# dohlee/diffab-pytorch

Hardware: AMD Instinct MI355X
Metric: CDR-residue denoise-steps/sec (K=128 patch) (higher is better)
Workload: dtype f32 (bf16x6 / fp16x3 split-precision products on the 16-bit matrix cores, fp32 accumulate; fp32-accurate, DESIGN section 4)

## Files before the change

diffab-pytorch_amd/csrc/ipa_persistent.hip:

```cpp
#include "common.h"
#include "denoiser_internal.h"
#define AT_STAMP_REALTIME 1
#include "ipa_attn_tile.h"
#include "proj_frames_h3_tile.h"
#include "rowgemm_h3_tile.h"
#include "mlp_chain_tile.h"

namespace diffab {

namespace {
constexpr size_t cmax(size_t a, size_t b) { return a > b ? a : b; }
constexpr size_t kModuleLdsBytes = cmax(cmax(ipa_attn_lds_bytes(8), static_cast<size_t>(kChainLdsBytes)),
                                        cmax(static_cast<size_t>(pjh3::PJ_LDS_BYTES), static_cast<size_t>(h3tile::lds_bytes<128>())));
constexpr size_t kXImageOffset = cmax(static_cast<size_t>(pjh3::PJ_LDS_BYTES), static_cast<size_t>(h3tile::lds_bytes<128>())) / 4;
static_assert(kXImageOffset * 4 + h3tile::y_lds_bytes<128>() <= kModuleLdsBytes, "module LDS: no room for the x image of the dense phases");
static_assert(kModuleLdsBytes <= 160 * 1024, "module LDS: one work-group per CU within gfx950's 160 KiB");
static_assert(kXImageOffset % 4 == 0, "x image: 16-byte aligned rows");

struct ModuleArgs {
  float* xa;
  float* xb;
  float* proj;
  float* feat;
  const float* pair;
  const float* esc;
  const int* ctx_of_row;
  const int* last_layer_rows;
  const float* R;
  const float* t;
  const char* planes;
  size_t layer_stride, pj_off, out_off, wis_off, small_off;
  unsigned long long* stamps;
  const float* emb_X;
  MlpChainSet emb, heads;
  int B, NL;
  int stagger_ticks, stagger_classes;
};
}

__device__ __forceinline__ int module_plan_word(const int* __restrict__ plan, const int idx) {
  int w;
  asm volatile("s_load_dword %0, %1, 0x0\n\ts_waitcnt lgkmcnt(0)" : "=s"(w) : "s"(plan + idx) : "memory");
  return w;
}

template <int KRES>
__global__ __launch_bounds__(512) void ipa_module_persistent_kernel(const ModuleArgs a) {
  extern __shared__ __attribute__((aligned(16))) float lds[];
  constexpr int K = KRES, NTILE = K / TI, DT = K / 128;
  static_assert(KRES == 128 || KRES == 256, "patch-resident module: K = 128 or 256");
  const int M = a.B * K;
  if (a.stagger_ticks > 0 && a.stagger_classes > 1) {
    const unsigned long long t0 = __builtin_amdgcn_s_memrealtime();
    const unsigned long long wait = static_cast<unsigned long long>((blockIdx.x >> 3) % a.stagger_classes) * a.stagger_ticks;
    while (__builtin_amdgcn_s_memrealtime() - t0 < wait) __builtin_amdgcn_s_sleep(32);
  }
  unsigned long long* pstamps = a.stamps ? a.stamps + static_cast<size_t>(a.B) * a.NL * NTILE * 64 : nullptr;
  auto pstamp = [&](int b, int l, int k) {
    if (pstamps != nullptr && threadIdx.x == 0) pstamps[(static_cast<size_t>(b) * a.NL + l) * 4 + k] = __builtin_amdgcn_s_memrealtime();
  };
#pragma unroll 1
  for (int b = blockIdx.x; b < a.B; b += gridDim.x) {
    if (a.emb_X != nullptr) {
#pragma unroll 1
      for (int dt = 0; dt < DT; ++dt) {
        int tid = threadIdx.x;
        asm volatile("" : "+v"(tid));
        chaintile::mlp_chain_tile(reinterpret_cast<__bf16*>(lds), tid, b * DT + dt, a.emb_X, 128, a.emb.c[0].planes[0], a.emb.c[0].planes[1],
                                  nullptr, a.emb.c[0].bias[0], a.emb.c[0].bias[1], nullptr, a.emb.c[0].bias_idx0, a.emb.c[0].bias_div0, 2, 128,
                                  a.xa, 128, M);
        asm volatile("s_waitcnt vmcnt(0)" ::: "memory");
        __syncthreads();
      }
    }
#pragma unroll 1
    for (int l = 0; l < a.NL; ++l) {
      const char* lp = a.planes + static_cast<size_t>(l) * a.layer_stride;
      const float* small = reinterpret_cast<const float*>(lp + a.small_off);
      const float* xin = (l & 1) ? a.xb : a.xa;
      float* xout = (l & 1) ? a.xa : a.xb;
      pstamp(b, l, 0);
#pragma unroll 1
      for (int dt = 0; dt < DT; ++dt) {
        int tid = threadIdx.x;
        asm volatile("" : "+v"(tid));
        if (KRES == 128) {
          if (l == 0) {
            float* xl = lds + kXImageOffset;
            for (int i = tid; i < 128 * 32; i += 512) {
              const int row = i >> 5, c4 = 4 * (i & 31);
              *reinterpret_cast<float4*>(xl + row * h3tile::Y_LDS_LD + c4) =
                  *reinterpret_cast<const float4*>(xin + (static_cast<int64_t>(b) * 128 + row) * 128 + c4);
            }
            __syncthreads();
          }
          pjh3::proj_frames_h3_tile<true, false, true, true>(reinterpret_cast<_Float16*>(lds), tid, b, 0, 1, nullptr,
                                                             reinterpret_cast<const _Float16*>(lp + a.pj_off),
                                                             reinterpret_cast<const float*>(lp + a.wis_off), a.R, a.t, a.proj, M, 0, 0, 0,
                                                             lds + kXImageOffset);
        } else {
          pjh3::proj_frames_h3_tile<true, false>(reinterpret_cast<_Float16*>(lds), tid, b * DT + dt, 0, 1, xin,
                                                 reinterpret_cast<const _Float16*>(lp + a.pj_off), reinterpret_cast<const float*>(lp + a.wis_off),
                                                 a.R, a.t, a.proj, M);
        }
        if (dt + 1 < DT) {
          asm volatile("s_waitcnt vmcnt(0)" ::: "memory");
          __syncthreads();
        }
      }
      asm volatile("s_waitcnt vmcnt(0)" ::: "memory");
      __syncthreads();
      pstamp(b, l, 1);
      const int* rows = l + 1 == a.NL ? a.last_layer_rows : nullptr;
      const int n_items = rows != nullptr ? module_plan_word(rows, b * (2 + NTILE)) : NTILE;
#pragma unroll 1
      for (int item = 0; item < n_items; ++item) {
        const int i0 = rows != nullptr ? module_plan_word(rows, b * (2 + NTILE) + 2 + item) : item * TI;
        ipa_attn_tile<8, (KRES > 128), true>(lds, b, i0, static_cast<unsigned>((b * a.NL + l) * NTILE + item), a.proj, a.pair, a.R, a.t, small,
                                             small + 512, a.feat, K / 128, a.stamps, a.esc, nullptr, nullptr, a.ctx_of_row);
        asm volatile("s_waitcnt vmcnt(0)" ::: "memory");
        __syncthreads();
      }
      pstamp(b, l, 2);
#pragma unroll 1
      for (int dt = 0; dt < DT; ++dt) {
        int tid = threadIdx.x;
        asm volatile("" : "+v"(tid));
        if (KRES == 128)
          h3tile::rowgemm128_h3_tile<false, 128, false, true>(reinterpret_cast<_Float16*>(lds), tid, b, a.feat, AF,
                                                              reinterpret_cast<const _Float16*>(lp + a.out_off),
                                                              reinterpret_cast<const float*>(lp + a.wis_off) + ANP, small + 576, nullptr, 0,
                                                              l + 1 == a.NL ? xout : nullptr, 128, M, AF, 0, nullptr, lds + kXImageOffset);
        else
          h3tile::rowgemm128_h3_tile<false, 128>(reinterpret_cast<_Float16*>(lds), tid, b * DT + dt, a.feat, AF,
                                                 reinterpret_cast<const _Float16*>(lp + a.out_off),
                                                 reinterpret_cast<const float*>(lp + a.wis_off) + ANP, small + 576, nullptr, 0, xout, 128, M, AF);
        if (dt + 1 < DT) {
          asm volatile("s_waitcnt vmcnt(0)" ::: "memory");
          __syncthreads();
        }
      }
      asm volatile("s_waitcnt vmcnt(0)" ::: "memory");
      __syncthreads();
      pstamp(b, l, 3);
    }
    if (a.emb_X != nullptr) {
      const float* xfin = (a.NL & 1) ? a.xb : a.xa;
#pragma unroll 1
      for (int hdt = 0; hdt < 3 * DT; ++hdt) {
        const int hd = hdt / DT, dt = hdt % DT;
        const unsigned hslabs =
            a.last_layer_rows != nullptr ? static_cast<unsigned>(module_plan_word(a.last_layer_rows, b * (2 + NTILE) + 1)) : ~0u;
        const unsigned tslabs = (hslabs >> (4 * dt)) & 15u;
        if (tslabs == 0) continue;
        int tid = threadIdx.x;
        asm volatile("" : "+v"(tid));
#define HSEL(f) (hd == 0 ? a.heads.c[0].f : hd == 1 ? a.heads.c[1].f : a.heads.c[2].f)
        chaintile::mlp_chain_tile<true>(reinterpret_cast<__bf16*>(lds), tid, b * DT + dt, xfin, 128, HSEL(planes[0]), HSEL(planes[1]), HSEL(planes[2]),
                                  HSEL(bias[0]), HSEL(bias[1]), HSEL(bias[2]), HSEL(bias_idx0), HSEL(bias_div0), 3, HSEL(n_out),
                                  hd == 0 ? a.heads.Y[0] : hd == 1 ? a.heads.Y[1] : a.heads.Y[2],
                                  hd == 0 ? a.heads.ldy[0] : hd == 1 ? a.heads.ldy[1] : a.heads.ldy[2], M, tslabs);
#undef HSEL
        asm volatile("s_waitcnt vmcnt(0)" ::: "memory");
        __syncthreads();
      }
      if (pstamps != nullptr && threadIdx.x == 0) pstamps[static_cast<size_t>(a.B) * a.NL * 4 + b] = __builtin_amdgcn_s_memrealtime();
    }
  }
}

namespace {
int g_stagger_ticks = 1000, g_stagger_classes = 8;
unsigned long long* g_module_stamps = nullptr;
}
void set_module_stagger(int ticks, int classes) {
  g_stagger_ticks = ticks;
  g_stagger_classes = classes;
}
void set_module_stamps(void* p) { g_module_stamps = static_cast<unsigned long long*>(p); }

bool ipa_module_persistent_supported(const diffab_dims* d) {
  return fast_path_supported(d) && (d->K == 128 || d->K == 256) && d->NL >= 1;
}

int launch_ipa_module_persistent(const diffab_dims* d, float* xa, float* xb, const float* R, const float* t, float* ws, const void* planes,
                                 const float* pair_planes, hipStream_t st, const float* emb_X, const MlpChainSet* emb,
                                 const MlpChainSet* heads, const int* ctx_of_row, int n_ctx, const int* last_layer_rows) {
  DIFFAB_REQUIRE(ipa_module_persistent_supported(d) && xa && xb && R && t && ws && planes && pair_planes, DIFFAB_ERR_ARG,
                 "ipa_module_persistent: unsupported operands");
  DIFFAB_REQUIRE((reinterpret_cast<uintptr_t>(last_layer_rows) & 3) == 0, DIFFAB_ERR_ARG,
                 "ipa_module_persistent: the row plan must be 4-byte aligned");
  const size_t rows = static_cast<size_t>(d->B) * d->K;
  ModuleArgs a{};
  a.xa = xa;
  a.xb = xb;
  a.proj = ws;
  a.feat = ws + rows * ANP;
  a.pair = pair_planes + 64;
  a.esc = pair_row_scales(d, pair_planes, n_ctx);
  a.ctx_of_row = ctx_of_row;
  a.last_layer_rows = last_layer_rows;
  a.R = R;
  a.t = t;
  a.planes = static_cast<const char*>(planes);
  a.layer_stride = ipa_layer_planes_bytes();
  a.pj_off = ipa_layer_h3_pj_offset();
  a.out_off = ipa_layer_h3_out_offset();
  a.wis_off = ipa_layer_h3_wis_offset();
  a.small_off = ipa_layer_small_offset();
  a.stamps = g_module_stamps;
  if (emb_X != nullptr) {
    DIFFAB_REQUIRE(emb && heads && d->D == 128 && (reinterpret_cast<uintptr_t>(emb_X) & 15) == 0, DIFFAB_ERR_ARG,
                   "ipa_module_persistent: the fused MLP phases need both chain sets");
    a.emb_X = emb_X;
    a.emb = *emb;
    a.heads = *heads;
  }
  a.B = d->B;
  a.NL = d->NL;
  a.stagger_ticks = g_stagger_ticks;
  a.stagger_classes = g_stagger_classes;
  int dev = 0, ncu = 256;
  if (hipGetDevice(&dev) == hipSuccess) (void)hipDeviceGetAttribute(&ncu, hipDeviceAttributeMultiprocessorCount, dev);
  const int grid = d->B < ncu ? d->B : ncu;
#define MODULE_LAUNCH(K_)                                                                                                       \
  do {                                                                                                                            \
    DIFFAB_HIP_CHECK(hipFuncSetAttribute(reinterpret_cast<const void*>(ipa_module_persistent_kernel<K_>),                         \
                                         hipFuncAttributeMaxDynamicSharedMemorySize, static_cast<int>(kModuleLdsBytes)));        \
    timer_begin(st);                                                                                                              \
    hipLaunchKernelGGL((ipa_module_persistent_kernel<K_>), dim3(grid), dim3(512), kModuleLdsBytes, st, a);                        \
    timer_end(st);                                                                                                                \
  } while (0)
  if (d->K == 128) MODULE_LAUNCH(128);
  else MODULE_LAUNCH(256);
#undef MODULE_LAUNCH
  DIFFAB_LAUNCH_CHECK();
  return DIFFAB_OK;
}

}
```

diffab-pytorch_amd/csrc/rowgemm_h3_tile.h:

```cpp
#pragma once
#include <hip/hip_runtime.h>

namespace diffab {
namespace h3tile {
typedef float f32x4 __attribute__((ext_vector_type(4)));
typedef _Float16 f16x8 __attribute__((ext_vector_type(8)));
typedef _Float16 f16x4 __attribute__((ext_vector_type(4)));
typedef float f32x16 __attribute__((ext_vector_type(16)));
constexpr int BK = 32;
constexpr int PART_CHUNKS = 2;

__device__ __forceinline__ int h3_off(int row, int slot) { return row * BK + 8 * (slot ^ ((row >> 2) & 3)); }
__device__ __forceinline__ void h3_scale(float m, float& s, float& is) {
  const int e = static_cast<int>((__float_as_uint(m) >> 23) & 255u);
  const bool ok = e >= 8 && e < 231;
  s = ok ? __uint_as_float(static_cast<unsigned>(127 + 7 + 127 - e) << 23) : 1.0f;
  is = ok ? __uint_as_float(static_cast<unsigned>(e - 7) << 23) : 1.0f;
}
__device__ __forceinline__ void split2(float x, _Float16& h1, _Float16& h2) {
  h1 = static_cast<_Float16>(x);
  h2 = static_cast<_Float16>(x - static_cast<float>(h1));
}
template <int ROWS>
constexpr int lds_bytes() { return 2 * 2 * (128 + ROWS) * BK * 2 + 2 * ROWS * 4; }

constexpr int Y_LDS_LD = 132;
template <int ROWS>
constexpr int y_lds_bytes() { return ROWS * Y_LDS_LD * 4; }

template <bool RELU, int ROWS, bool PARTIAL = false, bool Y_LDS = false>
__device__ __forceinline__ void rowgemm128_h3_tile(_Float16* h3_lds, int tid, int tile_m, const float* __restrict__ X, int ldx,
                                                   const _Float16* __restrict__ Wc, const float* __restrict__ wis, const float* __restrict__ bias,
                                                   const int64_t* __restrict__ bias_idx, int bias_div, float* __restrict__ Y, int ldy, int M, int Kd,
                                                   int c_begin = 0, float* __restrict__ part_out = nullptr, float* __restrict__ y_lds = nullptr) {
#define H3TILE_FENCE() asm volatile("" ::: "memory")
  constexpr int T = ROWS * 4, NRW = ROWS / 32;
  _Float16* Ws = h3_lds;
  _Float16* As = h3_lds + 2 * 2 * 128 * BK;
  float* Sx = reinterpret_cast<float*>(As + 2 * 2 * ROWS * BK);
  const int lane = tid & 63, wv = tid >> 6;
  const int l31 = lane & 31, hk = lane >> 5, rw = wv % NRW, cw = wv / NRW;
  const int m0 = tile_m * ROWS;
  const int nchunk = PARTIAL ? min(Kd / BK, c_begin + PART_CHUNKS) : Kd / BK;
  constexpr int WP = 1024 / T;
  int w_dst[WP];
#pragma unroll
  for (int i = 0; i < WP; ++i) {
    const int idx = tid + T * i, p = idx / 512, row = (idx % 512) >> 2, part = idx & 3;
    w_dst[i] = (p * 128) * BK + h3_off(row, part);
  }
  f32x4 wreg[2][WP];
  auto load_w = [&](int slot, int ch) {
    ch = ch < nchunk ? ch : nchunk - 1;
    const _Float16* src = Wc + static_cast<size_t>(ch) * (2 * 128 * BK) + tid * 8;
#pragma unroll
    for (int i = 0; i < WP; ++i) wreg[slot][i] = *reinterpret_cast<const f32x4*>(src + T * 8 * i);
  };
  auto store_w = [&](int slot, int buf) {
#pragma unroll
    for (int i = 0; i < WP; ++i) *reinterpret_cast<f32x4*>(Ws + buf * (2 * 128 * BK) + w_dst[i]) = wreg[slot][i];
  };
  const int xa_row = tid >> 3, xa_part = tid & 7;
  const float* xsrc[2];
  int x_dst[2];
#pragma unroll
  for (int j = 0; j < 2; ++j) {
    const int lrow = xa_row + (ROWS / 2) * j;
    int row = m0 + lrow;
    row = row < M ? row : M - 1;
    xsrc[j] = X + static_cast<int64_t>(row) * ldx + 4 * xa_part;
    x_dst[j] = h3_off(lrow, xa_part >> 1) + 4 * (xa_part & 1);
  }
  f32x4 xreg[4][2];
  auto load_x = [&](int slot, int ch) {
    ch = ch < nchunk ? ch : nchunk - 1;
#pragma unroll
    for (int j = 0; j < 2; ++j) xreg[slot][j] = *reinterpret_cast<const f32x4*>(xsrc[j] + ch * BK);
  };
  float sx_cur[2];
  auto pair_scale = [&](int slot_a, int slot_b, int pp) {
#pragma unroll
    for (int j = 0; j < 2; ++j) {
      const f32x4 va = xreg[slot_a][j], vb = xreg[slot_b][j];
      float m = fmaxf(fmaxf(fmaxf(fabsf(va[0]), fabsf(va[1])), fmaxf(fabsf(va[2]), fabsf(va[3]))),
                      fmaxf(fmaxf(fabsf(vb[0]), fabsf(vb[1])), fmaxf(fabsf(vb[2]), fabsf(vb[3]))));
      m = fmaxf(m, __shfl_xor(m, 1));
      m = fmaxf(m, __shfl_xor(m, 2));
      m = fmaxf(m, __shfl_xor(m, 4));
      float is;
      h3_scale(m, sx_cur[j], is);
      if (xa_part == 0) Sx[pp * ROWS + xa_row + (ROWS / 2) * j] = is;
    }
  };
  auto store_x = [&](int slot, int buf) {
#pragma unroll
    for (int j = 0; j < 2; ++j) {
      const f32x4 v = xreg[slot][j];
      f16x4 h1, h2;
#pragma unroll
      for (int c = 0; c < 4; ++c) {
        _Float16 a, b;
        split2(v[c] * sx_cur[j], a, b);
        h1[c] = a; h2[c] = b;
      }
      _Float16* dst = As + buf * (2 * ROWS * BK) + x_dst[j];
      *reinterpret_cast<f16x4*>(dst) = h1;
      *reinterpret_cast<f16x4*>(dst + ROWS * BK) = h2;
    }
  };
  f32x16 acc[2], tot[2];
#pragma unroll
  for (int tt = 0; tt < 2; ++tt)
#pragma unroll
    for (int r = 0; r < 16; ++r) acc[tt][r] = tot[tt][r] = 0.f;

#pragma unroll
  for (int c = 0; c < 4; ++c) load_x(c, c_begin + c);
  load_w(0, c_begin);
  load_w(1, c_begin + 1);
  H3TILE_FENCE();
  store_w(0, 0);
  pair_scale(0, 1, 0);
  store_x(0, 0);
  load_w(0, c_begin + 2);
  load_x(0, c_begin + 4);
  H3TILE_FENCE();
  __syncthreads();
  const int fx = (l31 >> 2) & 3;
  const int a_off = (32 * rw + l31) * BK, w_off = (64 * cw + l31) * BK;
  for (int ch0 = c_begin; ch0 < nchunk; ch0 += 4) {
#pragma unroll
    for (int u = 0; u < 4; ++u) {
      const int ch = ch0 + u, buf = u & 1;
      if (ch >= nchunk) break;
      const _Float16* al = As + buf * (2 * ROWS * BK) + a_off;
      const _Float16* wl = Ws + buf * (2 * 128 * BK) + w_off;
#pragma unroll
      for (int ks = 0; ks < 2; ++ks) {
        const int so = 8 * ((2 * ks + hk) ^ fx);
        f16x8 a[2], b[2][2];
#pragma unroll
        for (int p = 0; p < 2; ++p) {
          a[p] = *reinterpret_cast<const f16x8*>(al + (p * ROWS) * BK + so);
#pragma unroll
          for (int tt = 0; tt < 2; ++tt) b[tt][p] = *reinterpret_cast<const f16x8*>(wl + (p * 128 + 32 * tt) * BK + so);
        }
#pragma unroll
        for (int tt = 0; tt < 2; ++tt) acc[tt] = __builtin_amdgcn_mfma_f32_32x32x16_f16(a[1], b[tt][0], acc[tt], 0, 0, 0);
#pragma unroll
        for (int tt = 0; tt < 2; ++tt) acc[tt] = __builtin_amdgcn_mfma_f32_32x32x16_f16(a[0], b[tt][1], acc[tt], 0, 0, 0);
#pragma unroll
        for (int tt = 0; tt < 2; ++tt) acc[tt] = __builtin_amdgcn_mfma_f32_32x32x16_f16(a[0], b[tt][0], acc[tt], 0, 0, 0);
      }
      store_w((u + 1) & 1, buf ^ 1);
      if (u & 1) pair_scale((u + 1) & 3, (u + 2) & 3, ((u + 1) >> 1) & 1);
      store_x((u + 1) & 3, buf ^ 1);
      load_w((u + 1) & 1, ch + 3);
      load_x((u + 1) & 3, ch + 5);
      H3TILE_FENCE();
      if (u & 1) {
        f32x4 sx[4];
#pragma unroll
        for (int g = 0; g < 4; ++g) sx[g] = *reinterpret_cast<const f32x4*>(Sx + (u >> 1) * ROWS + 32 * rw + 8 * g + 4 * hk);
#pragma unroll
        for (int tt = 0; tt < 2; ++tt)
#pragma unroll
          for (int r = 0; r < 16; ++r) {
            tot[tt][r] = __builtin_fmaf(acc[tt][r], sx[r >> 2][r & 3], tot[tt][r]);
            acc[tt][r] = 0.f;
          }
      }
      __syncthreads();
    }
  }
  if (PARTIAL) {
#pragma unroll
    for (int tt = 0; tt < 2; ++tt)
#pragma unroll
      for (int r = 0; r < 16; ++r)
        part_out[(32 * rw + (r & 3) + 8 * (r >> 2) + 4 * hk) * 128 + 64 * cw + 32 * tt + l31] = tot[tt][r];
    return;
  }
  const bool table = bias_idx != nullptr || bias_div > 0;
  const bool y_global = !Y_LDS || Y != nullptr;
#pragma unroll
  for (int tt = 0; tt < 2; ++tt) {
    const int col = 64 * cw + 32 * tt + l31;
    const float wi = wis[col];
    float bv = (bias && !table) ? bias[col] : 0.0f;
#pragma unroll
    for (int r = 0; r < 16; ++r) {
      const int row = m0 + 32 * rw + (r & 3) + 8 * (r >> 2) + 4 * hk;
      if (row >= M) continue;
      if (table) {
        const int64_t bi = bias_idx ? bias_idx[row] : row / bias_div;
        bv = bias[bi * 128 + col];
      }
      float o = __builtin_fmaf(tot[tt][r], wi, bv);
      if (RELU) o = fmaxf(o, 0.f);
      if (Y_LDS) y_lds[(row - m0) * Y_LDS_LD + col] = o;
      if (y_global) Y[static_cast<int64_t>(row) * ldy + col] = o;
    }
  }
#undef H3TILE_FENCE
}
}
}
```

Measured before the change: 14.98 million.

## Restrict last-layer output GEMM to live 32-row slabs

On the last IPA layer, the output-projection row GEMM now takes a 4-bit mask of which 32-row slabs of the 128-row tile hold rows that are actually needed, read from the module plan. Waves are re-mapped so that each one computes a 32-column strip for up to two live slabs. X rows for dead slabs are neither converted nor stored, and the whole tile is skipped when the mask is empty. This cuts MFMA, LDS and global work when few CDR rows remain, at the cost of extra index logic and possibly uneven load across waves.

```diff
diff --git a/diffab-pytorch_amd/csrc/ipa_persistent.hip b/diffab-pytorch_amd/csrc/ipa_persistent.hip
--- a/diffab-pytorch_amd/csrc/ipa_persistent.hip
+++ b/diffab-pytorch_amd/csrc/ipa_persistent.hip
@@ -126,7 +126,12 @@
       for (int dt = 0; dt < DT; ++dt) {
         int tid = threadIdx.x;
         asm volatile("" : "+v"(tid));
-        if (KRES == 128)
+        if (KRES == 128 && rows != nullptr)
+          h3tile::rowgemm128_h3_tile<false, 128, false, false, true>(
+              reinterpret_cast<_Float16*>(lds), tid, b, a.feat, AF, reinterpret_cast<const _Float16*>(lp + a.out_off),
+              reinterpret_cast<const float*>(lp + a.wis_off) + ANP, small + 576, nullptr, 0, xout, 128, M, AF, 0, nullptr, nullptr,
+              static_cast<unsigned>(module_plan_word(rows, b * (2 + NTILE) + 1)));
+        else if (KRES == 128)
           h3tile::rowgemm128_h3_tile<false, 128, false, true>(reinterpret_cast<_Float16*>(lds), tid, b, a.feat, AF,
                                                               reinterpret_cast<const _Float16*>(lp + a.out_off),
                                                               reinterpret_cast<const float*>(lp + a.wis_off) + ANP, small + 576, nullptr, 0,
diff --git a/diffab-pytorch_amd/csrc/rowgemm_h3_tile.h b/diffab-pytorch_amd/csrc/rowgemm_h3_tile.h
--- a/diffab-pytorch_amd/csrc/rowgemm_h3_tile.h
+++ b/diffab-pytorch_amd/csrc/rowgemm_h3_tile.h
@@ -28,11 +28,14 @@
 template <int ROWS>
 constexpr int y_lds_bytes() { return ROWS * Y_LDS_LD * 4; }
 
-template <bool RELU, int ROWS, bool PARTIAL = false, bool Y_LDS = false>
+template <bool RELU, int ROWS, bool PARTIAL = false, bool Y_LDS = false, bool SLABS = false>
 __device__ __forceinline__ void rowgemm128_h3_tile(_Float16* h3_lds, int tid, int tile_m, const float* __restrict__ X, int ldx,
                                                    const _Float16* __restrict__ Wc, const float* __restrict__ wis, const float* __restrict__ bias,
                                                    const int64_t* __restrict__ bias_idx, int bias_div, float* __restrict__ Y, int ldy, int M, int Kd,
-                                                   int c_begin = 0, float* __restrict__ part_out = nullptr, float* __restrict__ y_lds = nullptr) {
+                                                   int c_begin = 0, float* __restrict__ part_out = nullptr, float* __restrict__ y_lds = nullptr,
+                                                   unsigned slabs = 15u) {
+  static_assert(!SLABS || (ROWS == 128 && !PARTIAL && !Y_LDS), "SLABS: one 128-row tile, complete sums, global output");
+  if (SLABS && (slabs & 15u) == 0) return;
 #define H3TILE_FENCE() asm volatile("" ::: "memory")
   constexpr int T = ROWS * 4, NRW = ROWS / 32;
   _Float16* Ws = h3_lds;
@@ -41,6 +44,20 @@
   const int lane = tid & 63, wv = tid >> 6;
   const int l31 = lane & 31, hk = lane >> 5, rw = wv % NRW, cw = wv / NRW;
   const int m0 = tile_m * ROWS;
+  int np = 2, rs[2] = {rw, rw}, cs = 0;
+  if (SLABS) {
+    const int wu = __builtin_amdgcn_readfirstlane(wv), hi = wu >> 2;
+    const unsigned sl = slabs & 15u;
+    const int n = __builtin_popcount(sl);
+    const int first = n <= 2 ? hi : 2 * hi;
+    np = n <= 2 ? (hi < n ? 1 : 0) : min(2, n - first);
+    unsigned m = sl;
+    for (int i = 0; i < first && np > 0; ++i) m &= m - 1;
+    rs[0] = np > 0 ? __builtin_ctz(m | 16u) & 3 : 0;
+    m &= m - 1;
+    rs[1] = np > 1 ? __builtin_ctz(m | 16u) & 3 : rs[0];
+    cs = wu & 3;
+  }
   const int nchunk = PARTIAL ? min(Kd / BK, c_begin + PART_CHUNKS) : Kd / BK;
   constexpr int WP = 1024 / T;
   int w_dst[WP];
@@ -63,10 +80,18 @@
   const int xa_row = tid >> 3, xa_part = tid & 7;
   const float* xsrc[2];
   int x_dst[2];
+  bool xw[2] = {true, true};
+  int x_alias = 0;
+  if (SLABS) {
+    const int xs = __builtin_amdgcn_readfirstlane(wv) >> 2;
+    xw[0] = (slabs >> xs) & 1u;
+    xw[1] = (slabs >> (2 + xs)) & 1u;
+    x_alias = 32 * (__builtin_ctz(slabs | 16u) & 3);
+  }
 #pragma unroll
   for (int j = 0; j < 2; ++j) {
     const int lrow = xa_row + (ROWS / 2) * j;
-    int row = m0 + lrow;
+    int row = m0 + (xw[j] ? lrow : x_alias + (lrow & 31));
     row = row < M ? row : M - 1;
     xsrc[j] = X + static_cast<int64_t>(row) * ldx + 4 * xa_part;
     x_dst[j] = h3_off(lrow, xa_part >> 1) + 4 * (xa_part & 1);
@@ -81,6 +106,7 @@
   auto pair_scale = [&](int slot_a, int slot_b, int pp) {
 #pragma unroll
     for (int j = 0; j < 2; ++j) {
+      if (!xw[j]) continue;
       const f32x4 va = xreg[slot_a][j], vb = xreg[slot_b][j];
       float m = fmaxf(fmaxf(fmaxf(fabsf(va[0]), fabsf(va[1])), fmaxf(fabsf(va[2]), fabsf(va[3]))),
                       fmaxf(fmaxf(fabsf(vb[0]), fabsf(vb[1])), fmaxf(fabsf(vb[2]), fabsf(vb[3]))));
@@ -95,6 +121,7 @@
   auto store_x = [&](int slot, int buf) {
 #pragma unroll
     for (int j = 0; j < 2; ++j) {
+      if (!xw[j]) continue;
       const f32x4 v = xreg[slot][j];
       f16x4 h1, h2;
 #pragma unroll
@@ -127,7 +154,8 @@
   H3TILE_FENCE();
   __syncthreads();
   const int fx = (l31 >> 2) & 3;
-  const int a_off = (32 * rw + l31) * BK, w_off = (64 * cw + l31) * BK;
+  const int a_off = (32 * rs[0] + l31) * BK, w_off = SLABS ? (32 * cs + l31) * BK : (64 * cw + l31) * BK;
+  const int a_off1 = (32 * rs[1] + l31) * BK;
   for (int ch0 = c_begin; ch0 < nchunk; ch0 += 4) {
 #pragma unroll
     for (int u = 0; u < 4; ++u) {
@@ -135,22 +163,56 @@
       if (ch >= nchunk) break;
       const _Float16* al = As + buf * (2 * ROWS * BK) + a_off;
       const _Float16* wl = Ws + buf * (2 * 128 * BK) + w_off;
-#pragma unroll
-      for (int ks = 0; ks < 2; ++ks) {
-        const int so = 8 * ((2 * ks + hk) ^ fx);
-        f16x8 a[2], b[2][2];
-#pragma unroll
-        for (int p = 0; p < 2; ++p) {
-          a[p] = *reinterpret_cast<const f16x8*>(al + (p * ROWS) * BK + so);
-#pragma unroll
-          for (int tt = 0; tt < 2; ++tt) b[tt][p] = *reinterpret_cast<const f16x8*>(wl + (p * 128 + 32 * tt) * BK + so);
+      if (SLABS) {
+        if (np > 0) {
+          f16x8 a[2][2], b[2][2];
+#pragma unroll
+          for (int ks = 0; ks < 2; ++ks) {
+            const int so = 8 * ((2 * ks + hk) ^ fx);
+#pragma unroll
+            for (int p = 0; p < 2; ++p) {
+              a[ks][p] = *reinterpret_cast<const f16x8*>(al + (p * ROWS) * BK + so);
+              b[ks][p] = *reinterpret_cast<const f16x8*>(wl + (p * 128) * BK + so);
+            }
+          }
+#pragma unroll
+          for (int ks = 0; ks < 2; ++ks) {
+            acc[0] = __builtin_amdgcn_mfma_f32_32x32x16_f16(a[ks][1], b[ks][0], acc[0], 0, 0, 0);
+            acc[0] = __builtin_amdgcn_mfma_f32_32x32x16_f16(a[ks][0], b[ks][1], acc[0], 0, 0, 0);
+            acc[0] = __builtin_amdgcn_mfma_f32_32x32x16_f16(a[ks][0], b[ks][0], acc[0], 0, 0, 0);
+          }
+          if (np > 1) {
+            const _Float16* al1 = As + buf * (2 * ROWS * BK) + a_off1;
+#pragma unroll
+            for (int ks = 0; ks < 2; ++ks)
+#pragma unroll
+              for (int p = 0; p < 2; ++p) a[ks][p] = *reinterpret_cast<const f16x8*>(al1 + (p * ROWS) * BK + 8 * ((2 * ks + hk) ^ fx));
+#pragma unroll
+            for (int ks = 0; ks < 2; ++ks) {
+              acc[1] = __builtin_amdgcn_mfma_f32_32x32x16_f16(a[ks][1], b[ks][0], acc[1], 0, 0, 0);
+              acc[1] = __builtin_amdgcn_mfma_f32_32x32x16_f16(a[ks][0], b[ks][1], acc[1], 0, 0, 0);
+              acc[1] = __builtin_amdgcn_mfma_f32_32x32x16_f16(a[ks][0], b[ks][0], acc[1], 0, 0, 0);
+            }
+          }
         }
-#pragma unroll
-        for (int tt = 0; tt < 2; ++tt) acc[tt] = __builtin_amdgcn_mfma_f32_32x32x16_f16(a[1], b[tt][0], acc[tt], 0, 0, 0);
-#pragma unroll
-        for (int tt = 0; tt < 2; ++tt) acc[tt] = __builtin_amdgcn_mfma_f32_32x32x16_f16(a[0], b[tt][1], acc[tt], 0, 0, 0);
-#pragma unroll
-        for (int tt = 0; tt < 2; ++tt) acc[tt] = __builtin_amdgcn_mfma_f32_32x32x16_f16(a[0], b[tt][0], acc[tt], 0, 0, 0);
+      } else {
+#pragma unroll
+        for (int ks = 0; ks < 2; ++ks) {
+          const int so = 8 * ((2 * ks + hk) ^ fx);
+          f16x8 a[2], b[2][2];
+#pragma unroll
+          for (int p = 0; p < 2; ++p) {
+            a[p] = *reinterpret_cast<const f16x8*>(al + (p * ROWS) * BK + so);
+#pragma unroll
+            for (int tt = 0; tt < 2; ++tt) b[tt][p] = *reinterpret_cast<const f16x8*>(wl + (p * 128 + 32 * tt) * BK + so);
+          }
+#pragma unroll
+          for (int tt = 0; tt < 2; ++tt) acc[tt] = __builtin_amdgcn_mfma_f32_32x32x16_f16(a[1], b[tt][0], acc[tt], 0, 0, 0);
+#pragma unroll
+          for (int tt = 0; tt < 2; ++tt) acc[tt] = __builtin_amdgcn_mfma_f32_32x32x16_f16(a[0], b[tt][1], acc[tt], 0, 0, 0);
+#pragma unroll
+          for (int tt = 0; tt < 2; ++tt) acc[tt] = __builtin_amdgcn_mfma_f32_32x32x16_f16(a[0], b[tt][0], acc[tt], 0, 0, 0);
+        }
       }
       store_w((u + 1) & 1, buf ^ 1);
       if (u & 1) pair_scale((u + 1) & 3, (u + 2) & 3, ((u + 1) >> 1) & 1);
@@ -160,15 +222,29 @@
       H3TILE_FENCE();
       if (u & 1) {
         f32x4 sx[4];
-#pragma unroll
-        for (int g = 0; g < 4; ++g) sx[g] = *reinterpret_cast<const f32x4*>(Sx + (u >> 1) * ROWS + 32 * rw + 8 * g + 4 * hk);
-#pragma unroll
-        for (int tt = 0; tt < 2; ++tt)
-#pragma unroll
-          for (int r = 0; r < 16; ++r) {
-            tot[tt][r] = __builtin_fmaf(acc[tt][r], sx[r >> 2][r & 3], tot[tt][r]);
-            acc[tt][r] = 0.f;
-          }
+        if (SLABS) {
+#pragma unroll
+          for (int tt = 0; tt < 2; ++tt)
+            if (tt < np) {
+#pragma unroll
+              for (int g = 0; g < 4; ++g) sx[g] = *reinterpret_cast<const f32x4*>(Sx + (u >> 1) * ROWS + 32 * rs[tt] + 8 * g + 4 * hk);
+#pragma unroll
+              for (int r = 0; r < 16; ++r) {
+                tot[tt][r] = __builtin_fmaf(acc[tt][r], sx[r >> 2][r & 3], tot[tt][r]);
+                acc[tt][r] = 0.f;
+              }
+            }
+        } else {
+#pragma unroll
+          for (int g = 0; g < 4; ++g) sx[g] = *reinterpret_cast<const f32x4*>(Sx + (u >> 1) * ROWS + 32 * rw + 8 * g + 4 * hk);
+#pragma unroll
+          for (int tt = 0; tt < 2; ++tt)
+#pragma unroll
+            for (int r = 0; r < 16; ++r) {
+              tot[tt][r] = __builtin_fmaf(acc[tt][r], sx[r >> 2][r & 3], tot[tt][r]);
+              acc[tt][r] = 0.f;
+            }
+        }
       }
       __syncthreads();
     }
@@ -185,12 +261,13 @@
   const bool y_global = !Y_LDS || Y != nullptr;
 #pragma unroll
   for (int tt = 0; tt < 2; ++tt) {
-    const int col = 64 * cw + 32 * tt + l31;
+    if (SLABS && tt >= np) continue;
+    const int col = SLABS ? 32 * cs + l31 : 64 * cw + 32 * tt + l31;
     const float wi = wis[col];
     float bv = (bias && !table) ? bias[col] : 0.0f;
 #pragma unroll
     for (int r = 0; r < 16; ++r) {
-      const int row = m0 + 32 * rw + (r & 3) + 8 * (r >> 2) + 4 * hk;
+      const int row = m0 + 32 * (SLABS ? rs[tt] : rw) + (r & 3) + 8 * (r >> 2) + 4 * hk;
       if (row >= M) continue;
       if (table) {
         const int64_t bi = bias_idx ? bias_idx[row] : row / bias_div;
```

Result: no change. 15.08 million (median of 6 runs) (+0.7%).
